# KdaiP/StableTTS

Hardware: NVIDIA B200
Metric: mel-frames/sec through CFM DiT estimator (ODE solve, all evaluations) (higher is better)
Workload: dtype f32 (split-bf16x3 tensor-core operands; FFN convs fp16 activations x fp16 hi/lo weights, 2 passes; fp32 accumulate)

## Files before the change

### profiles/trace_attention.py

```python
import os, sys, ctypes as C
sys.path.insert(0, os.path.dirname(os.path.dirname(os.path.abspath(__file__))))
import torch
from stabletts_b200 import CFMDecoder, _lib
dev = torch.device("cuda:0")
B = int(sys.argv[1]) if len(sys.argv) > 1 else 64
T = int(sys.argv[2]) if len(sys.argv) > 2 else 1000
m = CFMDecoder(80, 80, 256, 80, 1024, 4, 6, 3, 0.1, 256).eval().to(dev)
m.estimator._prepare(torch.zeros(1, device=dev), B, T, 0)
lib, h = _lib.load_library(), m.estimator._handle
s = torch.cuda.current_stream().cuda_stream
g = torch.Generator().manual_seed(3)
qkv = torch.randn(B, T, 768, generator=g).to(dev)
mask = torch.ones(B, T, device=dev)
out = torch.empty(B, T, 256, device=dev)
for _ in range(3):
    _lib.check(lib, h, lib.st_test_attention(h, qkv.data_ptr(), mask.data_ptr(), out.data_ptr(), B, T, s), "att")
torch.cuda.synchronize()
buf = (C.c_longlong * (32 * 16))()
assert lib.st_test_attention_trace(buf) == 0
tr = [[buf[j * 16 + k] for k in range(16)] for j in range(32)]
t0 = min(x for row in tr for x in row if x)
names = ["sm:wait_S", "sm:S_ready", "sm:max_done", "sm:xchg_done", "sm:exp_done", "sm:P_stored", "sm:arrived", "-",
         "mma:loop_top", "mma:P_ready", "mma:PV_issued", "mma:K_ready", "mma:S_issued"]
print("block | " + " | ".join(names))
for j, row in enumerate(tr):
    if not any(row): break
    print(f"{j:5d} | " + " | ".join(f"{(x - t0) if x else -1:8d}" for x in row[:13]))
print("softmax per block: wait_S, ld+max, xchg, exp, st, arrive ; mma: wait_P, issue_PV, wait_K, issue_S")
for j, row in enumerate(tr):
    if not any(row) or j == 0: continue
    s_ = row
    print(f"{j:5d} | S-wait {s_[1]-s_[0]:6d} ld+max {s_[2]-s_[1]:5d} xchg {s_[3]-s_[2]:5d} exp {s_[4]-s_[3]:5d} st {s_[5]-s_[4]:5d} arr {s_[6]-s_[5]:5d} "
          f"| period {s_[6]-tr[j-1][6]:6d} || P-wait {s_[9]-s_[8]:6d} PV {s_[10]-s_[9]:5d} K-wait {max(0,s_[11]-s_[10]):5d} S {max(0,s_[12]-s_[11]):5d}")
```

### stabletts_b200/csrc/attention_tc.cu

```cuda
#include "common.cuh"
#include "tc_ptx.cuh"
#include "gemm_epilogue.cuh"
#include <math_constants.h>
#include <mutex>
#include <string>
#include <cstring>
#include <cstdlib>
#include <cstdio>

namespace st {

bool tmap_encode_bf16(const void* ptr, int rank, uint64_t d0, uint64_t d1, uint64_t d2, uint32_t b0, uint32_t b1,
                      CUtensorMap* out);
const char* gemm_tc_last_error();

namespace {

using namespace ptx;

constexpr int AQ = 128;
constexpr int AK = 64;
constexpr int DH = 64;
constexpr int A_THREADS = 320;
constexpr int K_BYTES = AK * DH * 2;
constexpr int TMEM_COLS_ATT = 256;
constexpr float LAZY4 = 32.0f;

struct AttMaps { CUtensorMap q_hi, q_lo, kv_hi, kv_lo; };

struct AttParams {
    int BB, B, T, H, n_heads;
    const float* mask; const int* kvlen; const int* prefix;
    float* out_f32; bf16* out_hi; bf16* out_lo;
    const bf16* qkv_hi; const bf16* qkv_lo;
    long long* trace;
};

__device__ __forceinline__ float ex2_approx(float x) {
    float y;
    asm("ex2.approx.ftz.f32 %0, %1;" : "=f"(y) : "f"(x));
    return y;
}
__host__ __device__ constexpr uint32_t att_idesc(bool b_mn) { return make_idesc_bf16(128, 64) | (b_mn ? (1u << 16) : 0u); }

__global__ void rope_split_kernel(const float* __restrict__ qkv, const float* __restrict__ rope_cs, bf16* __restrict__ hi,
                                  bf16* __restrict__ lo, long rows, int T, int H) {
    const long i = (long)blockIdx.x * blockDim.x + threadIdx.x;
    const int H3 = 3 * H, half = H3 / 2;
    if (i >= rows * half) return;
    const long row = i / half;
    const int c = (int)(i % half) * 2;
    const int t = (int)(row % T);
    float x[2];
#pragma unroll
    for (int e = 0; e < 2; ++e) {
        const int n = c + e, d = n & 63;
        float v = qkv[row * H3 + n];
        if (n < 2 * H && d < 32) {
            const int j = d & 15;
            const float cs = rope_cs[((long)t * 16 + j) * 2], sn = rope_cs[((long)t * 16 + j) * 2 + 1];
            const float o = (d < 16) ? -qkv[row * H3 + n + 16] : qkv[row * H3 + n - 16];
            v = v * cs + o * sn;
        }
        if (n < H) v *= kQScale;
        x[e] = v;
    }
    uint32_t h2, l2;
    split_bf16x2(x[0], x[1], h2, l2);
    *reinterpret_cast<uint32_t*>(hi + row * H3 + c) = h2;
    *reinterpret_cast<uint32_t*>(lo + row * H3 + c) = l2;
}


__device__ __forceinline__ void umma_bf16_ts(uint32_t tmem_d, uint32_t tmem_a, uint64_t bdesc, uint32_t idesc, uint32_t accum) {
    asm volatile(
        "{\n\t"
        ".reg .pred p;\n\t"
        "setp.ne.b32 p, %4, 0;\n\t"
        "tcgen05.mma.cta_group::1.kind::f16 [%0], [%1], %2, %3, p;\n\t"
        "}" ::"r"(tmem_d), "r"(tmem_a), "l"(bdesc), "r"(idesc), "r"(accum) : "memory");
}

constexpr int ATT5_SMEM = 4 * K_BYTES + 4 * K_BYTES + 1024 + 2048 + 1024;

__global__ void __launch_bounds__(A_THREADS, 2)
attention_tc5_kernel(const __grid_constant__ AttMaps maps, const AttParams p) {
    extern __shared__ uint8_t smem_raw[];
    uint64_t* bars = reinterpret_cast<uint64_t*>(smem_raw);
    uint8_t* smem = reinterpret_cast<uint8_t*>((reinterpret_cast<uintptr_t>(smem_raw) + 160 + 1023) & ~uintptr_t(1023));
    uint8_t* sK = smem;
    uint8_t* sV = sK + 4 * K_BYTES;
    float* xmax = reinterpret_cast<float*>(sV + 4 * K_BYTES);
    float* xl = xmax + 2 * 2 * AQ;
    uint64_t *q_full = bars, *k_full = bars + 1 , *k_empty = bars + 3 , *v_full = bars + 5 ,
             *v_empty = bars + 7 , *pv_done = bars + 9, *s_full = bars + 10 , *p_full = bars + 12;
    uint32_t* tmem_slot = reinterpret_cast<uint32_t*>(bars + 13);
    if (reinterpret_cast<uint8_t*>(xl + 2 * AQ) > smem_raw + ATT5_SMEM) __trap();
    pdl_trigger(); pdl_wait();

    const int warp = threadIdx.x >> 5, lane = threadIdx.x & 31;
    const int bb = blockIdx.z, h = blockIdx.y, q0 = blockIdx.x * AQ;
    const int b = bb % p.B;
    const int kvlen = p.kvlen[b];
    const int ck = p.H + h * DH, cv = 2 * p.H + h * DH;

    if (q0 >= kvlen) {
        for (int i = threadIdx.x; i < AQ * (DH / 4); i += A_THREADS) {
            const int r = i / (DH / 4), c4 = (i % (DH / 4)) * 4, t = q0 + r;
            if (t < p.T) {
                const long o = ((long)bb * p.T + t) * p.H + h * DH + c4;
                if (p.out_f32) *reinterpret_cast<float4*>(p.out_f32 + o) = make_float4(0.f, 0.f, 0.f, 0.f);
                if (p.out_hi) { *reinterpret_cast<uint2*>(p.out_hi + o) = make_uint2(0, 0); *reinterpret_cast<uint2*>(p.out_lo + o) = make_uint2(0, 0); }
            }
        }
        return;
    }
    const int nb = (kvlen + AK - 1) / AK;
    long long* trc = (p.trace && blockIdx.x == 3 && blockIdx.y == 1 && blockIdx.z == 5) ? p.trace : nullptr;
#define TRC(j, slot) do { if (trc && (j) < 32) trc[(j) * 16 + (slot)] = clock64(); } while (0)

    if (warp == 0 && lane == 0) {
        for (int i = 0; i < 13; ++i) mbar_init(&bars[i], (i == 12 || i == 0) ? 8 : 1);
        mbar_fence_init();
    }
    if (warp == 1) tmem_alloc_1sm<TMEM_COLS_ATT>(tmem_slot);
    tc_fence_before();
    __syncthreads();
    tc_fence_after();
    const uint32_t tmem_base = *tmem_slot;
    const uint32_t tmem_O = tmem_base + 128, tmem_Qh = tmem_base + 192, tmem_Ql = tmem_base + 224;

    if (warp == 0) {
        if (elect_one()) {
            for (int j = 0; j < nb; ++j) {
                const int slot = j & 1;
                mbar_wait(&k_empty[slot], ((j >> 1) & 1) ^ 1);
                mbar_expect_tx(&k_full[slot], 2 * K_BYTES);
                tma_load_3d(&maps.kv_hi, &k_full[slot], sK + slot * 2 * K_BYTES, ck, j * AK, bb);
                tma_load_3d(&maps.kv_lo, &k_full[slot], sK + slot * 2 * K_BYTES + K_BYTES, ck, j * AK, bb);
                mbar_wait(&v_empty[slot], ((j >> 1) & 1) ^ 1);
                mbar_expect_tx(&v_full[slot], 2 * K_BYTES);
                tma_load_3d(&maps.kv_hi, &v_full[slot], sV + slot * 2 * K_BYTES, cv, j * AK, bb);
                tma_load_3d(&maps.kv_lo, &v_full[slot], sV + slot * 2 * K_BYTES + K_BYTES, cv, j * AK, bb);
            }
        }
    } else if (warp == 1) {
        constexpr uint32_t idesc_s = att_idesc(false), idesc_pv = att_idesc(true);
        constexpr uint64_t v_adv = (uint64_t)((16 * 128) >> 4);
        auto issue_S = [&](int j) {
            const int slot = j & 1;
            const uint64_t dKh = make_sw128_desc(smem_u32(sK + slot * 2 * K_BYTES));
            const uint64_t dKl = make_sw128_desc(smem_u32(sK + slot * 2 * K_BYTES + K_BYTES));
            const uint32_t tS = tmem_base + slot * 64;
#pragma unroll
            for (int k = 0; k < DH / 16; ++k) {
                const uint64_t adv = (uint64_t)(k * 2);
                umma_bf16_ts(tS, tmem_Ql + k * 8, dKh + adv, idesc_s, k != 0);
                umma_bf16_ts(tS, tmem_Qh + k * 8, dKl + adv, idesc_s, 1);
                umma_bf16_ts(tS, tmem_Qh + k * 8, dKh + adv, idesc_s, 1);
            }
            umma_commit(&k_empty[slot]);
            umma_commit(&s_full[slot]);
        };
        mbar_wait(q_full, 0);
        for (int j = 0; j < 2 && j < nb; ++j) {
            mbar_wait(&k_full[j], 0);
            tc_fence_after();
            if (elect_one()) issue_S(j);
            __syncwarp();
        }
        for (int j = 0; j < nb; ++j) {
            if (lane == 0) TRC(j, 8);
            mbar_wait(p_full, j & 1);
            mbar_wait(&v_full[j & 1], (j >> 1) & 1);
            tc_fence_after();
            if (lane == 0) TRC(j, 9);
            if (elect_one()) {
                const uint32_t tP = tmem_base + (j & 1) * 64;
                const uint64_t dVh = make_sw128_desc(smem_u32(sV + (j & 1) * 2 * K_BYTES));
                const uint64_t dVl = make_sw128_desc(smem_u32(sV + (j & 1) * 2 * K_BYTES + K_BYTES));
#pragma unroll
                for (int k = 0; k < AK / 16; ++k) {
                    const uint64_t va = (uint64_t)k * v_adv;
                    const uint32_t aH = tP + (k >> 1) * 32 + (k & 1) * 8, aL = aH + 16;
                    umma_bf16_ts(tmem_O, aL, dVh + va, idesc_pv, (j != 0) || (k != 0));
                    umma_bf16_ts(tmem_O, aH, dVl + va, idesc_pv, 1);
                    umma_bf16_ts(tmem_O, aH, dVh + va, idesc_pv, 1);
                }
                umma_commit(&v_empty[j & 1]);
                umma_commit(pv_done);
            }
            __syncwarp();
            if (lane == 0) TRC(j, 10);
            if (j + 2 < nb) {
                mbar_wait(&k_full[j & 1], ((j + 2) >> 1) & 1);
                tc_fence_after();
                if (lane == 0) TRC(j, 11);
                if (elect_one()) issue_S(j + 2);
                __syncwarp();
                if (lane == 0) TRC(j, 12);
            }
        }
    } else {
        const int wq = warp & 3;
        const int half = (warp - 2) >> 2;
        const int r = wq * 32 + lane;
        const int t = q0 + r;
        const uint32_t lane_addr = (uint32_t)(wq * 32) << 16;
        const uint32_t tOh = tmem_O + half * 32 + lane_addr;
        const int prefix = p.prefix[b];
        const float* mrow = p.mask + (long)b * p.T;
        uint32_t v[32];
        {
            const bf16* src = (half ? p.qkv_lo : p.qkv_hi) + ((long)bb * p.T + min(t, p.T - 1)) * (3 * p.H) + h * DH;
#pragma unroll
            for (int i = 0; i < 8; ++i) {
                uint4 q = make_uint4(0, 0, 0, 0);
                if (t < p.T) q = __ldg(reinterpret_cast<const uint4*>(src) + i);
                v[i * 4] = q.x; v[i * 4 + 1] = q.y; v[i * 4 + 2] = q.z; v[i * 4 + 3] = q.w;
            }
            tmem_st32((half ? tmem_Ql : tmem_Qh) + lane_addr, v);
            tmem_st_wait();
            tc_fence_before();
            __syncwarp();
            if (lane == 0) mbar_arrive(q_full);
        }
        float m_used = -CUDART_INF_F, l_run = 0.f;
        auto pair_sync = [wq]() {
            switch (wq) {
                case 0: asm volatile("bar.sync 1, 64;" ::: "memory"); break;
                case 1: asm volatile("bar.sync 2, 64;" ::: "memory"); break;
                case 2: asm volatile("bar.sync 3, 64;" ::: "memory"); break;
                default: asm volatile("bar.sync 4, 64;" ::: "memory"); break;
            }
        };

        for (int j = 0; j < nb; ++j) {
            const int k0 = j * AK + half * 32;
            const uint32_t tS = tmem_base + (j & 1) * 64 + half * 32 + lane_addr;
            const bool tr = warp == 2 && lane == 0;
            if (tr) TRC(j, 0);
            mbar_wait(&s_full[j & 1], (j >> 1) & 1);
            tc_fence_after();
            if (tr) TRC(j, 1);
            const bool need_mask = k0 + 32 > prefix;
            uint32_t bits = 0xffffffffu;
            if (need_mask) {
                const int ka = k0 + lane;
                bits = __ballot_sync(0xffffffffu, ka < kvlen && __ldg(mrow + min(ka, p.T - 1)) != 0.f);
            }
            bool waited_pv = (j == 0);
            auto load_scores = [&]() {
                tmem_ld32(tS, v);
                tmem_ld_wait();
                if (need_mask) {
#pragma unroll
                    for (int i = 0; i < 32; ++i) if (!((bits >> i) & 1u)) v[i] = 0xff800000u;
                }
            };
            load_scores();
            float c0 = -CUDART_INF_F, c1 = -CUDART_INF_F;
#pragma unroll
            for (int i = 0; i < 32; i += 4) {
                c0 = fmaxf(c0, fmaxf(__uint_as_float(v[i]), __uint_as_float(v[i + 1])));
                c1 = fmaxf(c1, fmaxf(__uint_as_float(v[i + 2]), __uint_as_float(v[i + 3])));
            }
            if (tr) TRC(j, 2);
            float* xm = xmax + (j & 1) * 2 * AQ;
            xm[half * AQ + r] = fmaxf(c0, c1);
            pair_sync();
            const float cand = fmaxf(fmaxf(c0, c1), xm[(half ^ 1) * AQ + r]);
            if (tr) TRC(j, 3);
            if (__any_sync(0xffffffffu, cand > m_used + LAZY4)) {
                const float m_new = (cand > m_used + LAZY4) ? cand : m_used;
                const float factor = (m_new == -CUDART_INF_F || m_used == -CUDART_INF_F) ? 1.f : ex2_approx(m_used - m_new);
                l_run *= factor;
                if (j > 0) {
                    mbar_wait(pv_done, (j - 1) & 1);
                    tc_fence_after();
                    waited_pv = true;
                    tmem_ld32(tOh, v);
                    tmem_ld_wait();
#pragma unroll
                    for (int i = 0; i < 32; ++i) v[i] = __float_as_uint(__uint_as_float(v[i]) * factor);
                    tmem_st32(tOh, v);
                    tmem_st_wait();
                    load_scores();
                }
                m_used = m_new;
            }
            uint32_t hw[16], lw[16];
            {
                const float m_eff = (m_used == -CUDART_INF_F) ? 0.f : m_used;
                float ps0 = 0.f, ps1 = 0.f, ps2 = 0.f, ps3 = 0.f;
#pragma unroll
                for (int i = 0; i < 32; i += 4) {
                    const float p0 = ex2_approx(__uint_as_float(v[i]) - m_eff), p1 = ex2_approx(__uint_as_float(v[i + 1]) - m_eff);
                    const float p2 = ex2_approx(__uint_as_float(v[i + 2]) - m_eff), p3 = ex2_approx(__uint_as_float(v[i + 3]) - m_eff);
                    ps0 += p0; ps1 += p1; ps2 += p2; ps3 += p3;
                    split_bf16x2(p0, p1, hw[i / 2], lw[i / 2]);
                    split_bf16x2(p2, p3, hw[i / 2 + 1], lw[i / 2 + 1]);
                }
                l_run += (ps0 + ps1) + (ps2 + ps3);
            }
            if (tr) TRC(j, 4);
            {
                uint32_t pk[32];
#pragma unroll
                for (int i = 0; i < 16; ++i) { pk[i] = hw[i]; pk[16 + i] = lw[i]; }
                tmem_st32(tS, pk);
                tmem_st_wait();
            }
            if (tr) TRC(j, 5);
            if (!waited_pv) mbar_wait(pv_done, (j - 1) & 1);
            tc_fence_before();
            __syncwarp();
            if (lane == 0) mbar_arrive(p_full);
            if (tr) TRC(j, 6);
        }
        mbar_wait(pv_done, (nb - 1) & 1);
        tc_fence_after();
        xl[half * AQ + r] = l_run;
        pair_sync();
        const float lsum = l_run + xl[(half ^ 1) * AQ + r];
        const bool valid = t < p.T && mrow[min(t, p.T - 1)] != 0.f && lsum > 0.f;
        const float inv = valid ? 1.0f / lsum : 0.f;
        tmem_ld32(tOh, v);
        tmem_ld_wait();
        if (t < p.T) {
            const long o = ((long)bb * p.T + t) * p.H + h * DH + half * 32;
#pragma unroll
            for (int c = 0; c < 4; ++c) {
                float f[8];
#pragma unroll
                for (int e = 0; e < 8; ++e) f[e] = __uint_as_float(v[c * 8 + e]) * inv;
                const long oc = o + c * 8;
                if (p.out_f32) {
                    *reinterpret_cast<float4*>(p.out_f32 + oc) = make_float4(f[0], f[1], f[2], f[3]);
                    *reinterpret_cast<float4*>(p.out_f32 + oc + 4) = make_float4(f[4], f[5], f[6], f[7]);
                }
                if (p.out_hi) {
                    uint32_t h4[4], l4[4];
#pragma unroll
                    for (int e = 0; e < 4; ++e) split_bf16x2(f[2 * e], f[2 * e + 1], h4[e], l4[e]);
                    *reinterpret_cast<uint4*>(p.out_hi + oc) = make_uint4(h4[0], h4[1], h4[2], h4[3]);
                    *reinterpret_cast<uint4*>(p.out_lo + oc) = make_uint4(l4[0], l4[1], l4[2], l4[3]);
                }
            }
        }
        tc_fence_before();
    }
    tc_fence_before();
    __syncthreads();
    if (warp == 1) {
        tc_fence_after();
        tmem_dealloc_1sm<TMEM_COLS_ATT>(tmem_base);
    }
#undef TRC
}

std::mutex g_att_mu;
long long* g_att_trace = nullptr;
std::atomic<uint64_t> g_att_attr5{0};
std::string g_att_err;

}

const char* attention_tc_last_error() { return g_att_err.c_str(); }

int attention_tc_read_trace(long long* host_out) {
    if (!g_att_trace) return 1;
    return cudaMemcpy(host_out, g_att_trace, 32 * 16 * sizeof(long long), cudaMemcpyDeviceToHost) == cudaSuccess ? 0 : 1;
}

cudaError_t launch_rope_split(const float* qkv, const float* rope_cs, bf16* hi, bf16* lo, int BB, int T, int H, cudaStream_t s) {
    const long rows = (long)BB * T, n = rows * (3 * H / 2);
    if (n == 0) return cudaSuccess;
    rope_split_kernel<<<(unsigned)((n + 255) / 256), 256, 0, s>>>(qkv, rope_cs, hi, lo, rows, T, H);
    return cudaGetLastError();
}

cudaError_t launch_attention_tc(const AttnArgs& a, cudaStream_t s) {
    std::lock_guard<std::mutex> lk(g_att_mu);
    if (a.H != a.n_heads * DH) return cudaErrorInvalidValue;
    if (a.BB == 0 || a.T == 0) return cudaSuccess;
    if (!a.qkv_hi || !a.qkv_lo) { g_att_err = "split qkv planes missing"; return cudaErrorInvalidValue; }
    AttMaps maps;
    const uint64_t C3 = 3 * (uint64_t)a.H;
    bool ok = true;
    ok = ok && tmap_encode_bf16(a.qkv_hi, 3, C3, (uint64_t)a.T, (uint64_t)a.BB, DH, AQ, &maps.q_hi);
    ok = ok && tmap_encode_bf16(a.qkv_lo, 3, C3, (uint64_t)a.T, (uint64_t)a.BB, DH, AQ, &maps.q_lo);
    ok = ok && tmap_encode_bf16(a.qkv_hi, 3, C3, (uint64_t)a.T, (uint64_t)a.BB, DH, AK, &maps.kv_hi);
    ok = ok && tmap_encode_bf16(a.qkv_lo, 3, C3, (uint64_t)a.T, (uint64_t)a.BB, DH, AK, &maps.kv_lo);
    if (!ok) { g_att_err = gemm_tc_last_error(); return cudaErrorInvalidValue; }
    AttParams p;
    p.BB = a.BB; p.B = a.B; p.T = a.T; p.H = a.H; p.n_heads = a.n_heads;
    p.mask = a.mask; p.kvlen = a.kvlen; p.prefix = a.prefix;
    p.out_f32 = a.out_f32; p.out_hi = a.out_hi; p.out_lo = a.out_lo;
    p.qkv_hi = a.qkv_hi; p.qkv_lo = a.qkv_lo;
    p.trace = nullptr;
    if (getenv("STABLETTS_B200_ATT_TRACE")) {
        if (!g_att_trace) { cudaMalloc(&g_att_trace, 32 * 16 * sizeof(long long)); }
        cudaMemsetAsync(g_att_trace, 0, 32 * 16 * sizeof(long long), s);
        p.trace = g_att_trace;
    }
    {
        cudaError_t e = ensure_dyn_smem(attention_tc5_kernel, ATT5_SMEM, g_att_attr5);
        if (e != cudaSuccess) { g_att_err = "cudaFuncSetAttribute failed for the attention kernels"; return e; }
    }
    dim3 grid((a.T + AQ - 1) / AQ, a.n_heads, a.BB);
    return launch_k(attention_tc5_kernel, grid, dim3(A_THREADS), (size_t)ATT5_SMEM, s, maps, p);
}

}
```

Before: 604,200.

## Make attention kernel persistent over tiles with cross-tile K/V and Q prefetch

Turns the attention kernel into a persistent one. The grid is capped at two CTAs per SM and each CTA loops over (q-tile, head, batch) tiles. Barrier phases carry a global block counter across tiles, so the TMA producer keeps streaming K/V for the next tile, and the softmax warps load the next Q before finishing the current tile's epilogue. This is meant to hide per-tile prologue/epilogue latency and the cost of launching and setting up CTAs. Tracing moves into a template parameter so its branches drop out of the default build, and a pipe throughput probe is added. The cost is extra complexity in barrier parity and a static tile assignment that may balance poorly when kvlen varies.

Result: no change. 606,100, median of 6 (+0.3%).

```diff
diff --git a/profiles/pipe_probe.cu b/profiles/pipe_probe.cu
--- /dev/null
+++ b/profiles/pipe_probe.cu
@@ -0,0 +1,72 @@
+#include <cstdio>
+#include <cstdint>
+#include <cuda_runtime.h>
+
+constexpr int ITERS = 4096;
+constexpr int CHAINS = 8;
+
+template <int KIND>
+__global__ void __launch_bounds__(1024, 1) probe(float* sink, long long* clk, float seed) {
+    float x[CHAINS];
+    uint32_t u[CHAINS];
+#pragma unroll
+    for (int c = 0; c < CHAINS; ++c) { x[c] = seed * (c + 1) * 1e-3f - 4.f; u[c] = __float_as_uint(x[c]); }
+    __syncthreads();
+    const long long t0 = clock64();
+#pragma unroll 4
+    for (int i = 0; i < ITERS; ++i) {
+#pragma unroll
+        for (int c = 0; c < CHAINS; ++c) {
+            if (KIND == 0) {
+                asm volatile("ex2.approx.ftz.f32 %0, %0;" : "+f"(x[c]));
+            } else if (KIND == 1) {
+                asm volatile("cvt.rn.bf16x2.f32 %0, %1, %0;" : "+r"(u[c]) : "f"(x[c]));
+            } else if (KIND == 2) {
+                if (c & 1) asm volatile("cvt.rn.bf16x2.f32 %0, %1, %0;" : "+r"(u[c]) : "f"(x[c]));
+                else asm volatile("ex2.approx.ftz.f32 %0, %0;" : "+f"(x[c]));
+            } else {
+                asm volatile("fma.rn.f32 %0, %0, 0f3F7FFFFF, 0f33800000;" : "+f"(x[c]));
+            }
+        }
+    }
+    __syncthreads();
+    const long long t1 = clock64();
+    float acc = 0.f;
+#pragma unroll
+    for (int c = 0; c < CHAINS; ++c) acc += x[c] + __uint_as_float(u[c]);
+    if (acc == 12345.f) sink[threadIdx.x] = acc;
+    if (threadIdx.x == 0) clk[blockIdx.x] = t1 - t0;
+}
+
+int main() {
+    int dev = 0, sms = 0;
+    cudaDeviceGetAttribute(&sms, cudaDevAttrMultiProcessorCount, dev);
+    cudaDeviceProp prop;
+    cudaGetDeviceProperties(&prop, dev);
+    float* sink; long long* clk;
+    cudaMalloc(&sink, 1024 * sizeof(float));
+    cudaMalloc(&clk, sms * sizeof(long long));
+    long long* h = new long long[sms];
+    const char* names[4] = {"ex2.approx.ftz.f32", "cvt.rn.bf16x2.f32", "ex2+cvt interleaved 1:1", "fma.rn.f32"};
+    printf("{\"device\": \"%s\", \"sms\": %d, \"threads_per_sm\": 1024, \"results\": [", prop.name, sms);
+    for (int k = 0; k < 4; ++k) {
+        for (int rep = 0; rep < 2; ++rep) {
+            switch (k) {
+                case 0: probe<0><<<sms, 1024>>>(sink, clk, 1.f); break;
+                case 1: probe<1><<<sms, 1024>>>(sink, clk, 1.f); break;
+                case 2: probe<2><<<sms, 1024>>>(sink, clk, 1.f); break;
+                default: probe<3><<<sms, 1024>>>(sink, clk, 1.f); break;
+            }
+        }
+        if (cudaDeviceSynchronize() != cudaSuccess) { printf("]}\n"); fprintf(stderr, "probe failed\n"); return 1; }
+        cudaMemcpy(h, clk, sms * sizeof(long long), cudaMemcpyDeviceToHost);
+        long long mn = h[0], mx = h[0], sum = 0;
+        for (int i = 0; i < sms; ++i) { mn = h[i] < mn ? h[i] : mn; mx = h[i] > mx ? h[i] : mx; sum += h[i]; }
+        const double warp_instr = 32.0 * ITERS * CHAINS;
+        printf("%s{\"stream\": \"%s\", \"clk_mean\": %.0f, \"warp_instr_per_clk_per_sm\": %.3f, "
+               "\"min_clk\": %lld, \"max_clk\": %lld}", k ? ", " : "", names[k], (double)sum / sms,
+               warp_instr / ((double)sum / sms), mn, mx);
+    }
+    printf("]}\n");
+    return 0;
+}
diff --git a/profiles/pipe_probe.py b/profiles/pipe_probe.py
--- /dev/null
+++ b/profiles/pipe_probe.py
@@ -0,0 +1,17 @@
+import json, os, subprocess, sys, tempfile
+
+HERE = os.path.dirname(os.path.abspath(__file__))
+nvcc = os.environ.get("NVCC", "/usr/local/cuda/bin/nvcc")
+with tempfile.TemporaryDirectory() as d:
+    exe = os.path.join(d, "pipe_probe")
+    subprocess.run([nvcc, "-gencode", "arch=compute_100a,code=sm_100a", "-O3", "-o", exe,
+                    os.path.join(HERE, "pipe_probe.cu")], check=True)
+    res = json.loads(subprocess.run([exe], check=True, capture_output=True, text=True).stdout)
+r = {x["stream"]: x["warp_instr_per_clk_per_sm"] for x in res["results"]}
+a, b, both = r["ex2.approx.ftz.f32"], r["cvt.rn.bf16x2.f32"], r["ex2+cvt interleaved 1:1"]
+res["shared_pipe_prediction"] = round(2 / (1 / a + 1 / b), 3)
+res["separate_pipe_prediction"] = round(2 * min(a, b), 3)
+print(json.dumps(res, indent=1))
+if len(sys.argv) > 1:
+    with open(sys.argv[1], "w") as f:
+        json.dump(res, f, indent=1)
diff --git a/profiles/trace_attention.py b/profiles/trace_attention.py
--- a/profiles/trace_attention.py
+++ b/profiles/trace_attention.py
@@ -26,9 +26,14 @@
 for j, row in enumerate(tr):
     if not any(row): break
     print(f"{j:5d} | " + " | ".join(f"{(x - t0) if x else -1:8d}" for x in row[:13]))
-print("softmax per block: wait_S, ld+max, xchg, exp, st, arrive ; mma: wait_P, issue_PV, wait_K, issue_S")
-for j, row in enumerate(tr):
-    if not any(row) or j == 0: continue
-    s_ = row
-    print(f"{j:5d} | S-wait {s_[1]-s_[0]:6d} ld+max {s_[2]-s_[1]:5d} xchg {s_[3]-s_[2]:5d} exp {s_[4]-s_[3]:5d} st {s_[5]-s_[4]:5d} arr {s_[6]-s_[5]:5d} "
-          f"| period {s_[6]-tr[j-1][6]:6d} || P-wait {s_[9]-s_[8]:6d} PV {s_[10]-s_[9]:5d} K-wait {max(0,s_[11]-s_[10]):5d} S {max(0,s_[12]-s_[11]):5d}")
+start, tstart, q_in, o_done, o_stored = tr[0][13], tr[0][14], tr[0][15], tr[1][13], tr[1][14]
+nb = max(j for j, row in enumerate(tr) if row[6]) + 1
+first_s, last_arr = tr[0][1], tr[nb - 1][6]
+if all((start, tstart, q_in, o_done, o_stored)):
+    life = o_stored - tstart
+    pro, loop, epi = first_s - tstart, last_arr - first_s, o_stored - last_arr
+    print(f"CTA start -> tile start {tstart - start} clk; tile {life} clk over {nb} key blocks: ->Q in TMEM {q_in - tstart}, "
+          f"->S_0 ready {first_s - q_in} | loop {loop} ({loop / max(nb - 1, 1):.0f} per block after the first) | "
+          f"last P->O complete {o_done - last_arr}, ->O stored {o_stored - o_done}")
+    print(f"outside the loop: before {pro} ({100 * pro / life:.1f} %), after {epi} ({100 * epi / life:.1f} %), "
+          f"together {100 * (pro + epi) / life:.1f} % of the tile's time")
diff --git a/stabletts_b200/csrc/attention_tc.cu b/stabletts_b200/csrc/attention_tc.cu
--- a/stabletts_b200/csrc/attention_tc.cu
+++ b/stabletts_b200/csrc/attention_tc.cu
@@ -83,6 +83,7 @@
 
 constexpr int ATT5_SMEM = 4 * K_BYTES + 4 * K_BYTES + 1024 + 2048 + 1024;
 
+template <bool kTrace>
 __global__ void __launch_bounds__(A_THREADS, 2)
 attention_tc5_kernel(const __grid_constant__ AttMaps maps, const AttParams p) {
     extern __shared__ uint8_t smem_raw[];
@@ -96,28 +97,25 @@
              *v_empty = bars + 7 , *pv_done = bars + 9, *s_full = bars + 10 , *p_full = bars + 12;
     uint32_t* tmem_slot = reinterpret_cast<uint32_t*>(bars + 13);
     if (reinterpret_cast<uint8_t*>(xl + 2 * AQ) > smem_raw + ATT5_SMEM) __trap();
+    const long long t_start = kTrace ? clock64() : 0;
     pdl_trigger(); pdl_wait();
 
     const int warp = threadIdx.x >> 5, lane = threadIdx.x & 31;
-    const int bb = blockIdx.z, h = blockIdx.y, q0 = blockIdx.x * AQ;
-    const int b = bb % p.B;
-    const int kvlen = p.kvlen[b];
-    const int ck = p.H + h * DH, cv = 2 * p.H + h * DH;
-
-    if (q0 >= kvlen) {
-        for (int i = threadIdx.x; i < AQ * (DH / 4); i += A_THREADS) {
-            const int r = i / (DH / 4), c4 = (i % (DH / 4)) * 4, t = q0 + r;
-            if (t < p.T) {
-                const long o = ((long)bb * p.T + t) * p.H + h * DH + c4;
-                if (p.out_f32) *reinterpret_cast<float4*>(p.out_f32 + o) = make_float4(0.f, 0.f, 0.f, 0.f);
-                if (p.out_hi) { *reinterpret_cast<uint2*>(p.out_hi + o) = make_uint2(0, 0); *reinterpret_cast<uint2*>(p.out_lo + o) = make_uint2(0, 0); }
-            }
-        }
-        return;
-    }
-    const int nb = (kvlen + AK - 1) / AK;
-    long long* trc = (p.trace && blockIdx.x == 3 && blockIdx.y == 1 && blockIdx.z == 5) ? p.trace : nullptr;
-#define TRC(j, slot) do { if (trc && (j) < 32) trc[(j) * 16 + (slot)] = clock64(); } while (0)
+    const int ntq = (p.T + AQ - 1) / AQ, tiles = ntq * p.n_heads * p.BB;
+    struct Tile { int q0, h, bb, kvlen, nb; };
+    auto tile_at = [&](int t) {
+        Tile c;
+        c.q0 = (t % ntq) * AQ; c.h = (t / ntq) % p.n_heads; c.bb = t / (ntq * p.n_heads);
+        c.kvlen = p.kvlen[c.bb % p.B];
+        c.nb = c.q0 < c.kvlen ? (c.kvlen + AK - 1) / AK : 0;
+        return c;
+    };
+    long long* trc = nullptr;
+#define TRC(j, slot) do { if (kTrace && trc && (j) < 32) trc[(j) * 16 + (slot)] = clock64(); } while (0)
+    const bool tr0 = kTrace && threadIdx.x == 64;
+    auto trace_tile = [&](const Tile& c) {
+        if (kTrace) trc = (p.trace && c.q0 == 3 * AQ && c.h == 1 && c.bb == 5) ? p.trace : nullptr;
+    };
 
     if (warp == 0 && lane == 0) {
         for (int i = 0; i < 13; ++i) mbar_init(&bars[i], (i == 12 || i == 0) ? 8 : 1);
@@ -132,23 +130,28 @@
 
     if (warp == 0) {
         if (elect_one()) {
-            for (int j = 0; j < nb; ++j) {
-                const int slot = j & 1;
-                mbar_wait(&k_empty[slot], ((j >> 1) & 1) ^ 1);
-                mbar_expect_tx(&k_full[slot], 2 * K_BYTES);
-                tma_load_3d(&maps.kv_hi, &k_full[slot], sK + slot * 2 * K_BYTES, ck, j * AK, bb);
-                tma_load_3d(&maps.kv_lo, &k_full[slot], sK + slot * 2 * K_BYTES + K_BYTES, ck, j * AK, bb);
-                mbar_wait(&v_empty[slot], ((j >> 1) & 1) ^ 1);
-                mbar_expect_tx(&v_full[slot], 2 * K_BYTES);
-                tma_load_3d(&maps.kv_hi, &v_full[slot], sV + slot * 2 * K_BYTES, cv, j * AK, bb);
-                tma_load_3d(&maps.kv_lo, &v_full[slot], sV + slot * 2 * K_BYTES + K_BYTES, cv, j * AK, bb);
+            uint32_t g = 0;
+            for (int t = blockIdx.x; t < tiles; t += gridDim.x) {
+                const Tile c = tile_at(t);
+                const int ck = p.H + c.h * DH, cv = 2 * p.H + c.h * DH;
+                for (int j = 0; j < c.nb; ++j, ++g) {
+                    const int slot = g & 1;
+                    mbar_wait(&k_empty[slot], ((g >> 1) & 1) ^ 1);
+                    mbar_expect_tx(&k_full[slot], 2 * K_BYTES);
+                    tma_load_3d(&maps.kv_hi, &k_full[slot], sK + slot * 2 * K_BYTES, ck, j * AK, c.bb);
+                    tma_load_3d(&maps.kv_lo, &k_full[slot], sK + slot * 2 * K_BYTES + K_BYTES, ck, j * AK, c.bb);
+                    mbar_wait(&v_empty[slot], ((g >> 1) & 1) ^ 1);
+                    mbar_expect_tx(&v_full[slot], 2 * K_BYTES);
+                    tma_load_3d(&maps.kv_hi, &v_full[slot], sV + slot * 2 * K_BYTES, cv, j * AK, c.bb);
+                    tma_load_3d(&maps.kv_lo, &v_full[slot], sV + slot * 2 * K_BYTES + K_BYTES, cv, j * AK, c.bb);
+                }
             }
         }
     } else if (warp == 1) {
         constexpr uint32_t idesc_s = att_idesc(false), idesc_pv = att_idesc(true);
         constexpr uint64_t v_adv = (uint64_t)((16 * 128) >> 4);
-        auto issue_S = [&](int j) {
-            const int slot = j & 1;
+        auto issue_S = [&](uint32_t gg) {
+            const int slot = gg & 1;
             const uint64_t dKh = make_sw128_desc(smem_u32(sK + slot * 2 * K_BYTES));
             const uint64_t dKl = make_sw128_desc(smem_u32(sK + slot * 2 * K_BYTES + K_BYTES));
             const uint32_t tS = tmem_base + slot * 64;
@@ -162,61 +165,67 @@
             umma_commit(&k_empty[slot]);
             umma_commit(&s_full[slot]);
         };
-        mbar_wait(q_full, 0);
-        for (int j = 0; j < 2 && j < nb; ++j) {
-            mbar_wait(&k_full[j], 0);
-            tc_fence_after();
-            if (elect_one()) issue_S(j);
-            __syncwarp();
-        }
-        for (int j = 0; j < nb; ++j) {
-            if (lane == 0) TRC(j, 8);
-            mbar_wait(p_full, j & 1);
-            mbar_wait(&v_full[j & 1], (j >> 1) & 1);
-            tc_fence_after();
-            if (lane == 0) TRC(j, 9);
-            if (elect_one()) {
-                const uint32_t tP = tmem_base + (j & 1) * 64;
-                const uint64_t dVh = make_sw128_desc(smem_u32(sV + (j & 1) * 2 * K_BYTES));
-                const uint64_t dVl = make_sw128_desc(smem_u32(sV + (j & 1) * 2 * K_BYTES + K_BYTES));
-#pragma unroll
-                for (int k = 0; k < AK / 16; ++k) {
-                    const uint64_t va = (uint64_t)k * v_adv;
-                    const uint32_t aH = tP + (k >> 1) * 32 + (k & 1) * 8, aL = aH + 16;
-                    umma_bf16_ts(tmem_O, aL, dVh + va, idesc_pv, (j != 0) || (k != 0));
-                    umma_bf16_ts(tmem_O, aH, dVl + va, idesc_pv, 1);
-                    umma_bf16_ts(tmem_O, aH, dVh + va, idesc_pv, 1);
-                }
-                umma_commit(&v_empty[j & 1]);
-                umma_commit(pv_done);
-            }
-            __syncwarp();
-            if (lane == 0) TRC(j, 10);
-            if (j + 2 < nb) {
-                mbar_wait(&k_full[j & 1], ((j + 2) >> 1) & 1);
+        uint32_t g = 0, tl = 0;
+        for (int t = blockIdx.x; t < tiles; t += gridDim.x) {
+            const Tile c = tile_at(t);
+            if (c.nb == 0) continue;
+            trace_tile(c);
+            mbar_wait(q_full, tl & 1);
+            for (int j = 0; j < 2 && j < c.nb; ++j) {
+                mbar_wait(&k_full[(g + j) & 1], ((g + j) >> 1) & 1);
                 tc_fence_after();
-                if (lane == 0) TRC(j, 11);
-                if (elect_one()) issue_S(j + 2);
+                if (elect_one()) issue_S(g + j);
                 __syncwarp();
-                if (lane == 0) TRC(j, 12);
-            }
+            }
+            for (int j = 0; j < c.nb; ++j) {
+                const uint32_t gj = g + j;
+                if (lane == 0) TRC(j, 8);
+                mbar_wait(p_full, gj & 1);
+                mbar_wait(&v_full[gj & 1], (gj >> 1) & 1);
+                tc_fence_after();
+                if (lane == 0) TRC(j, 9);
+                if (elect_one()) {
+                    const uint32_t tP = tmem_base + (gj & 1) * 64;
+                    const uint64_t dVh = make_sw128_desc(smem_u32(sV + (gj & 1) * 2 * K_BYTES));
+                    const uint64_t dVl = make_sw128_desc(smem_u32(sV + (gj & 1) * 2 * K_BYTES + K_BYTES));
+#pragma unroll
+                    for (int k = 0; k < AK / 16; ++k) {
+                        const uint64_t va = (uint64_t)k * v_adv;
+                        const uint32_t aH = tP + (k >> 1) * 32 + (k & 1) * 8, aL = aH + 16;
+                        umma_bf16_ts(tmem_O, aL, dVh + va, idesc_pv, (j != 0) || (k != 0));
+                        umma_bf16_ts(tmem_O, aH, dVl + va, idesc_pv, 1);
+                        umma_bf16_ts(tmem_O, aH, dVh + va, idesc_pv, 1);
+                    }
+                    umma_commit(&v_empty[gj & 1]);
+                    umma_commit(pv_done);
+                }
+                __syncwarp();
+                if (lane == 0) TRC(j, 10);
+                if (j + 2 < c.nb) {
+                    mbar_wait(&k_full[gj & 1], ((gj + 2) >> 1) & 1);
+                    tc_fence_after();
+                    if (lane == 0) TRC(j, 11);
+                    if (elect_one()) issue_S(gj + 2);
+                    __syncwarp();
+                    if (lane == 0) TRC(j, 12);
+                }
+            }
+            g += c.nb; ++tl;
         }
     } else {
         const int wq = warp & 3;
         const int half = (warp - 2) >> 2;
         const int r = wq * 32 + lane;
-        const int t = q0 + r;
         const uint32_t lane_addr = (uint32_t)(wq * 32) << 16;
         const uint32_t tOh = tmem_O + half * 32 + lane_addr;
-        const int prefix = p.prefix[b];
-        const float* mrow = p.mask + (long)b * p.T;
         uint32_t v[32];
-        {
-            const bf16* src = (half ? p.qkv_lo : p.qkv_hi) + ((long)bb * p.T + min(t, p.T - 1)) * (3 * p.H) + h * DH;
+        auto load_q = [&](const Tile& c) {
+            const int tq = c.q0 + r;
+            const bf16* src = (half ? p.qkv_lo : p.qkv_hi) + ((long)c.bb * p.T + min(tq, p.T - 1)) * (3 * p.H) + c.h * DH;
 #pragma unroll
             for (int i = 0; i < 8; ++i) {
                 uint4 q = make_uint4(0, 0, 0, 0);
-                if (t < p.T) q = __ldg(reinterpret_cast<const uint4*>(src) + i);
+                if (tq < p.T) q = __ldg(reinterpret_cast<const uint4*>(src) + i);
                 v[i * 4] = q.x; v[i * 4 + 1] = q.y; v[i * 4 + 2] = q.z; v[i * 4 + 3] = q.w;
             }
             tmem_st32((half ? tmem_Ql : tmem_Qh) + lane_addr, v);
@@ -224,8 +233,11 @@
             tc_fence_before();
             __syncwarp();
             if (lane == 0) mbar_arrive(q_full);
-        }
-        float m_used = -CUDART_INF_F, l_run = 0.f;
+        };
+        auto next_live = [&](int t) {
+            for (t += gridDim.x; t < tiles; t += gridDim.x) if (tile_at(t).nb) break;
+            return t;
+        };
         auto pair_sync = [wq]() {
             switch (wq) {
                 case 0: asm volatile("bar.sync 1, 64;" ::: "memory"); break;
@@ -234,121 +246,158 @@
                 default: asm volatile("bar.sync 4, 64;" ::: "memory"); break;
             }
         };
-
-        for (int j = 0; j < nb; ++j) {
-            const int k0 = j * AK + half * 32;
-            const uint32_t tS = tmem_base + (j & 1) * 64 + half * 32 + lane_addr;
-            const bool tr = warp == 2 && lane == 0;
-            if (tr) TRC(j, 0);
-            mbar_wait(&s_full[j & 1], (j >> 1) & 1);
+        uint32_t g = 0;
+        bool q_ready = false;
+        for (int t = blockIdx.x; t < tiles; t += gridDim.x) {
+            const Tile c = tile_at(t);
+            if (c.nb == 0) {
+                for (int i = threadIdx.x - 64; i < AQ * (DH / 4); i += A_THREADS - 64) {
+                    const int rr = i / (DH / 4), c4 = (i % (DH / 4)) * 4, tq = c.q0 + rr;
+                    if (tq < p.T) {
+                        const long o = ((long)c.bb * p.T + tq) * p.H + c.h * DH + c4;
+                        if (p.out_f32) *reinterpret_cast<float4*>(p.out_f32 + o) = make_float4(0.f, 0.f, 0.f, 0.f);
+                        if (p.out_hi) { *reinterpret_cast<uint2*>(p.out_hi + o) = make_uint2(0, 0); *reinterpret_cast<uint2*>(p.out_lo + o) = make_uint2(0, 0); }
+                    }
+                }
+                continue;
+            }
+            trace_tile(c);
+            if (tr0 && trc) trc[13] = t_start;
+            if (tr0) TRC(0, 14);
+            if (!q_ready) load_q(c);
+            if (tr0) TRC(0, 15);
+            const int tn = next_live(t);
+            if (tn < tiles) {
+                const Tile cn = tile_at(tn);
+                const bf16* src = (half ? p.qkv_lo : p.qkv_hi) + ((long)cn.bb * p.T + min(cn.q0 + r, p.T - 1)) * (3 * p.H) + cn.h * DH;
+                asm volatile("prefetch.global.L2 [%0];" :: "l"(src));
+            }
+            const int nb = c.nb, kvlen = c.kvlen, tq = c.q0 + r, b = c.bb % p.B;
+            const int prefix = p.prefix[b];
+            const float* mrow = p.mask + (long)b * p.T;
+            float m_used = -CUDART_INF_F, l_run = 0.f;
+
+            for (int j = 0; j < nb; ++j) {
+                const uint32_t gj = g + j;
+                const int k0 = j * AK + half * 32;
+                const uint32_t tS = tmem_base + (gj & 1) * 64 + half * 32 + lane_addr;
+                const bool tr = warp == 2 && lane == 0;
+                if (tr) TRC(j, 0);
+                mbar_wait(&s_full[gj & 1], (gj >> 1) & 1);
+                tc_fence_after();
+                if (tr) TRC(j, 1);
+                const bool need_mask = k0 + 32 > prefix;
+                uint32_t bits = 0xffffffffu;
+                if (need_mask) {
+                    const int ka = k0 + lane;
+                    bits = __ballot_sync(0xffffffffu, ka < kvlen && __ldg(mrow + min(ka, p.T - 1)) != 0.f);
+                }
+                bool waited_pv = (j == 0);
+                auto load_scores = [&]() {
+                    tmem_ld32(tS, v);
+                    tmem_ld_wait();
+                    if (need_mask) {
+#pragma unroll
+                        for (int i = 0; i < 32; ++i) if (!((bits >> i) & 1u)) v[i] = 0xff800000u;
+                    }
+                };
+                load_scores();
+                float c0 = -CUDART_INF_F, c1 = -CUDART_INF_F;
+#pragma unroll
+                for (int i = 0; i < 32; i += 4) {
+                    c0 = fmaxf(c0, fmaxf(__uint_as_float(v[i]), __uint_as_float(v[i + 1])));
+                    c1 = fmaxf(c1, fmaxf(__uint_as_float(v[i + 2]), __uint_as_float(v[i + 3])));
+                }
+                if (tr) TRC(j, 2);
+                float* xm = xmax + (j & 1) * 2 * AQ;
+                xm[half * AQ + r] = fmaxf(c0, c1);
+                pair_sync();
+                const float cand = fmaxf(fmaxf(c0, c1), xm[(half ^ 1) * AQ + r]);
+                if (tr) TRC(j, 3);
+                if (__any_sync(0xffffffffu, cand > m_used + LAZY4)) {
+                    const float m_new = (cand > m_used + LAZY4) ? cand : m_used;
+                    const float factor = (m_new == -CUDART_INF_F || m_used == -CUDART_INF_F) ? 1.f : ex2_approx(m_used - m_new);
+                    l_run *= factor;
+                    if (j > 0) {
+                        mbar_wait(pv_done, (gj - 1) & 1);
+                        tc_fence_after();
+                        waited_pv = true;
+                        tmem_ld32(tOh, v);
+                        tmem_ld_wait();
+#pragma unroll
+                        for (int i = 0; i < 32; ++i) v[i] = __float_as_uint(__uint_as_float(v[i]) * factor);
+                        tmem_st32(tOh, v);
+                        tmem_st_wait();
+                        load_scores();
+                    }
+                    m_used = m_new;
+                }
+                uint32_t hw[16], lw[16];
+                {
+                    const float m_eff = (m_used == -CUDART_INF_F) ? 0.f : m_used;
+                    float ps0 = 0.f, ps1 = 0.f, ps2 = 0.f, ps3 = 0.f;
+#pragma unroll
+                    for (int i = 0; i < 32; i += 4) {
+                        const float p0 = ex2_approx(__uint_as_float(v[i]) - m_eff), p1 = ex2_approx(__uint_as_float(v[i + 1]) - m_eff);
+                        const float p2 = ex2_approx(__uint_as_float(v[i + 2]) - m_eff), p3 = ex2_approx(__uint_as_float(v[i + 3]) - m_eff);
+                        ps0 += p0; ps1 += p1; ps2 += p2; ps3 += p3;
+                        split_bf16x2(p0, p1, hw[i / 2], lw[i / 2]);
+                        split_bf16x2(p2, p3, hw[i / 2 + 1], lw[i / 2 + 1]);
+                    }
+                    l_run += (ps0 + ps1) + (ps2 + ps3);
+                }
+                if (tr) TRC(j, 4);
+                {
+                    uint32_t pk[32];
+#pragma unroll
+                    for (int i = 0; i < 16; ++i) { pk[i] = hw[i]; pk[16 + i] = lw[i]; }
+                    tmem_st32(tS, pk);
+                    tmem_st_wait();
+                }
+                if (tr) TRC(j, 5);
+                if (!waited_pv) mbar_wait(pv_done, (gj - 1) & 1);
+                tc_fence_before();
+                __syncwarp();
+                if (lane == 0) mbar_arrive(p_full);
+                if (tr) TRC(j, 6);
+            }
+            g += nb;
+            q_ready = tn < tiles;
+            if (q_ready) load_q(tile_at(tn));
+            mbar_wait(pv_done, (g - 1) & 1);
             tc_fence_after();
-            if (tr) TRC(j, 1);
-            const bool need_mask = k0 + 32 > prefix;
-            uint32_t bits = 0xffffffffu;
-            if (need_mask) {
-                const int ka = k0 + lane;
-                bits = __ballot_sync(0xffffffffu, ka < kvlen && __ldg(mrow + min(ka, p.T - 1)) != 0.f);
-            }
-            bool waited_pv = (j == 0);
-            auto load_scores = [&]() {
-                tmem_ld32(tS, v);
-                tmem_ld_wait();
-                if (need_mask) {
-#pragma unroll
-                    for (int i = 0; i < 32; ++i) if (!((bits >> i) & 1u)) v[i] = 0xff800000u;
-                }
-            };
-            load_scores();
-            float c0 = -CUDART_INF_F, c1 = -CUDART_INF_F;
-#pragma unroll
-            for (int i = 0; i < 32; i += 4) {
-                c0 = fmaxf(c0, fmaxf(__uint_as_float(v[i]), __uint_as_float(v[i + 1])));
-                c1 = fmaxf(c1, fmaxf(__uint_as_float(v[i + 2]), __uint_as_float(v[i + 3])));
-            }
-            if (tr) TRC(j, 2);
-            float* xm = xmax + (j & 1) * 2 * AQ;
-            xm[half * AQ + r] = fmaxf(c0, c1);
+            if (tr0) TRC(1, 13);
+            xl[half * AQ + r] = l_run;
             pair_sync();
-            const float cand = fmaxf(fmaxf(c0, c1), xm[(half ^ 1) * AQ + r]);
-            if (tr) TRC(j, 3);
-            if (__any_sync(0xffffffffu, cand > m_used + LAZY4)) {
-                const float m_new = (cand > m_used + LAZY4) ? cand : m_used;
-                const float factor = (m_new == -CUDART_INF_F || m_used == -CUDART_INF_F) ? 1.f : ex2_approx(m_used - m_new);
-                l_run *= factor;
-                if (j > 0) {
-                    mbar_wait(pv_done, (j - 1) & 1);
-                    tc_fence_after();
-                    waited_pv = true;
-                    tmem_ld32(tOh, v);
-                    tmem_ld_wait();
-#pragma unroll
-                    for (int i = 0; i < 32; ++i) v[i] = __float_as_uint(__uint_as_float(v[i]) * factor);
-                    tmem_st32(tOh, v);
-                    tmem_st_wait();
-                    load_scores();
-                }
-                m_used = m_new;
-            }
-            uint32_t hw[16], lw[16];
-            {
-                const float m_eff = (m_used == -CUDART_INF_F) ? 0.f : m_used;
-                float ps0 = 0.f, ps1 = 0.f, ps2 = 0.f, ps3 = 0.f;
-#pragma unroll
-                for (int i = 0; i < 32; i += 4) {
-                    const float p0 = ex2_approx(__uint_as_float(v[i]) - m_eff), p1 = ex2_approx(__uint_as_float(v[i + 1]) - m_eff);
-                    const float p2 = ex2_approx(__uint_as_float(v[i + 2]) - m_eff), p3 = ex2_approx(__uint_as_float(v[i + 3]) - m_eff);
-                    ps0 += p0; ps1 += p1; ps2 += p2; ps3 += p3;
-                    split_bf16x2(p0, p1, hw[i / 2], lw[i / 2]);
-                    split_bf16x2(p2, p3, hw[i / 2 + 1], lw[i / 2 + 1]);
-                }
-                l_run += (ps0 + ps1) + (ps2 + ps3);
-            }
-            if (tr) TRC(j, 4);
-            {
-                uint32_t pk[32];
-#pragma unroll
-                for (int i = 0; i < 16; ++i) { pk[i] = hw[i]; pk[16 + i] = lw[i]; }
-                tmem_st32(tS, pk);
-                tmem_st_wait();
-            }
-            if (tr) TRC(j, 5);
-            if (!waited_pv) mbar_wait(pv_done, (j - 1) & 1);
+            const float lsum = l_run + xl[(half ^ 1) * AQ + r];
+            const bool valid = tq < p.T && mrow[min(tq, p.T - 1)] != 0.f && lsum > 0.f;
+            const float inv = valid ? 1.0f / lsum : 0.f;
+            tmem_ld32(tOh, v);
+            tmem_ld_wait();
+            if (tq < p.T) {
+                const long o = ((long)c.bb * p.T + tq) * p.H + c.h * DH + half * 32;
+#pragma unroll
+                for (int cc = 0; cc < 4; ++cc) {
+                    float f[8];
+#pragma unroll
+                    for (int e = 0; e < 8; ++e) f[e] = __uint_as_float(v[cc * 8 + e]) * inv;
+                    const long oc = o + cc * 8;
+                    if (p.out_f32) {
+                        *reinterpret_cast<float4*>(p.out_f32 + oc) = make_float4(f[0], f[1], f[2], f[3]);
+                        *reinterpret_cast<float4*>(p.out_f32 + oc + 4) = make_float4(f[4], f[5], f[6], f[7]);
+                    }
+                    if (p.out_hi) {
+                        uint32_t h4[4], l4[4];
+#pragma unroll
+                        for (int e = 0; e < 4; ++e) split_bf16x2(f[2 * e], f[2 * e + 1], h4[e], l4[e]);
+                        *reinterpret_cast<uint4*>(p.out_hi + oc) = make_uint4(h4[0], h4[1], h4[2], h4[3]);
+                        *reinterpret_cast<uint4*>(p.out_lo + oc) = make_uint4(l4[0], l4[1], l4[2], l4[3]);
+                    }
+                }
+            }
             tc_fence_before();
-            __syncwarp();
-            if (lane == 0) mbar_arrive(p_full);
-            if (tr) TRC(j, 6);
+            if (tr0) TRC(1, 14);
         }
-        mbar_wait(pv_done, (nb - 1) & 1);
-        tc_fence_after();
-        xl[half * AQ + r] = l_run;
-        pair_sync();
-        const float lsum = l_run + xl[(half ^ 1) * AQ + r];
-        const bool valid = t < p.T && mrow[min(t, p.T - 1)] != 0.f && lsum > 0.f;
-        const float inv = valid ? 1.0f / lsum : 0.f;
-        tmem_ld32(tOh, v);
-        tmem_ld_wait();
-        if (t < p.T) {
-            const long o = ((long)bb * p.T + t) * p.H + h * DH + half * 32;
-#pragma unroll
-            for (int c = 0; c < 4; ++c) {
-                float f[8];
-#pragma unroll
-                for (int e = 0; e < 8; ++e) f[e] = __uint_as_float(v[c * 8 + e]) * inv;
-                const long oc = o + c * 8;
-                if (p.out_f32) {
-                    *reinterpret_cast<float4*>(p.out_f32 + oc) = make_float4(f[0], f[1], f[2], f[3]);
-                    *reinterpret_cast<float4*>(p.out_f32 + oc + 4) = make_float4(f[4], f[5], f[6], f[7]);
-                }
-                if (p.out_hi) {
-                    uint32_t h4[4], l4[4];
-#pragma unroll
-                    for (int e = 0; e < 4; ++e) split_bf16x2(f[2 * e], f[2 * e + 1], h4[e], l4[e]);
-                    *reinterpret_cast<uint4*>(p.out_hi + oc) = make_uint4(h4[0], h4[1], h4[2], h4[3]);
-                    *reinterpret_cast<uint4*>(p.out_lo + oc) = make_uint4(l4[0], l4[1], l4[2], l4[3]);
-                }
-            }
-        }
-        tc_fence_before();
     }
     tc_fence_before();
     __syncthreads();
@@ -361,7 +410,7 @@
 
 std::mutex g_att_mu;
 long long* g_att_trace = nullptr;
-std::atomic<uint64_t> g_att_attr5{0};
+std::atomic<uint64_t> g_att_attr5{0}, g_att_attr5_trace{0};
 std::string g_att_err;
 
 }
@@ -405,11 +454,18 @@
         p.trace = g_att_trace;
     }
     {
-        cudaError_t e = ensure_dyn_smem(attention_tc5_kernel, ATT5_SMEM, g_att_attr5);
+        cudaError_t e = p.trace ? ensure_dyn_smem(attention_tc5_kernel<true>, ATT5_SMEM, g_att_attr5_trace)
+                                : ensure_dyn_smem(attention_tc5_kernel<false>, ATT5_SMEM, g_att_attr5);
         if (e != cudaSuccess) { g_att_err = "cudaFuncSetAttribute failed for the attention kernels"; return e; }
     }
-    dim3 grid((a.T + AQ - 1) / AQ, a.n_heads, a.BB);
-    return launch_k(attention_tc5_kernel, grid, dim3(A_THREADS), (size_t)ATT5_SMEM, s, maps, p);
-}
-
-}
+    const long tiles = (long)((a.T + AQ - 1) / AQ) * a.n_heads * a.BB;
+    int dev = 0, sms = 0;
+    cudaGetDevice(&dev);
+    cudaDeviceGetAttribute(&sms, cudaDevAttrMultiProcessorCount, dev);
+    if (sms <= 0) { g_att_err = "multiprocessor count unavailable"; return cudaErrorInvalidValue; }
+    const dim3 grid((unsigned)std::min<long>(tiles, 2L * sms));
+    return p.trace ? launch_k(attention_tc5_kernel<true>, grid, dim3(A_THREADS), (size_t)ATT5_SMEM, s, maps, p)
+                   : launch_k(attention_tc5_kernel<false>, grid, dim3(A_THREADS), (size_t)ATT5_SMEM, s, maps, p);
+}
+
+}
```
